# ceselder/pacman-marl-2025

Measured on AMD Instinct MI355X. Metric: env-steps/s (4-agent smallCapture), higher is better.
Workload: dtype u32; 1 GPU; smallCapture.lay 2v2, 16384 envs/GPU, gymPacMan tick (self_play), length 300, auto-reset, uniform random actions (Philox seed 1234), 4 observations/env-tick; envs_per_gpu=16384, layout=smallCapture, obs_dtype=float32, obs_bytes_per_elem=4, parallelism=env-sharded x1, no data-path collective

## Files before the change

### pacman-marl-2025_amd/csrc/pmx_step.hip

```cpp
#include <algorithm>
#include <cstdlib>

#include <hip/hip_ext.h>

#include "pmx_device.h"

#define PMX_MAX_H_LDS 32

namespace {

struct Env {
    uint32_t xy[4];
    int dir[4], pac[4], scared[4], carry[4], ret[4];
    uint32_t capw[2];
    int score, steps;
    uint32_t ticks;
    uint32_t self_after[4];
};

struct Acc {
    double red_r, blue_r;
    int red_sc, blue_sc, sc_total;
    int n_red, n_blue;
};
// ... 475 lines not shown
    st[(size_t)PMX_W_CAPS(c.H, 1) * N + env] = e.capw[1];
}
template <int K0, int K1>
__device__ __forceinline__ void wide_group(const uint32_t *lds_rows, int n_rows, int word0, int sub, int q4, uint32_t *dst, int N)
{
    if constexpr (K0 < K1) {
        const int r = 4 * K0 + sub;
        const uint4 v = *reinterpret_cast<const uint4 *>(lds_rows + (r < n_rows ? r : 0) * PMX_RULE_BLOCK + q4);
        wide_group<K0 + 1, K1>(lds_rows, n_rows, word0, sub, q4, dst, N);
        if (r < n_rows) *reinterpret_cast<uint4 *>(dst + (size_t)(word0 + r) * N) = v;
    }
}
template <int HB, int NW>
__device__ __forceinline__ void store_words_wide(const Ctx &c, const uint32_t (&w)[NW], uint32_t *st, int N)
{
    const int lane = threadIdx.x, sub = lane >> 4, q4 = 4 * (lane & 15);
    uint32_t *dst = st + (size_t)blockIdx.x * PMX_RULE_BLOCK + q4;
#pragma unroll
    for (int i = 0; i < NW; ++i) c.stg[i * PMX_RULE_BLOCK + lane] = w[i];
    __builtin_amdgcn_fence(__ATOMIC_ACQ_REL, "wavefront");
    __builtin_amdgcn_wave_barrier();
    constexpr int KR = HB / 4, KW = (NW + 3) / 4;
    wide_group<0, KR>(c.rows0, c.H, 0, sub, q4, dst, N);
    wide_group<0, KW>(c.stg, NW, c.H, sub, q4, dst, N);
    __builtin_amdgcn_fence(__ATOMIC_ACQ_REL, "wavefront");
    __builtin_amdgcn_wave_barrier();
}
template <int HB>
__device__ __forceinline__ void store_snapshot_wide(const Env &e, const Ctx &c, uint32_t *st, int N)
{
    uint32_t w[10];
#pragma unroll
    for (int i = 0; i < 4; ++i) { w[i] = pack_a(e, i); w[4 + i] = pack_b(e, i); }
    w[8] = e.capw[0]; w[9] = e.capw[1];
    store_words_wide<HB, 10>(c, w, st, N);
}
template <int HB>
__device__ __forceinline__ void store_env_wide(const Env &e, const Ctx &c, uint32_t *st, int N)
{
    uint32_t w[13];
#pragma unroll
    for (int i = 0; i < 4; ++i) { w[i] = pack_a(e, i); w[4 + i] = pack_b(e, i); }
    w[8] = e.capw[0]; w[9] = e.capw[1];
    w[10] = (uint32_t)e.score; w[11] = (uint32_t)e.steps; w[12] = e.ticks;
    store_words_wide<HB, 13>(c, w, st, N);
}
template <int HB = 0>
__device__ __forceinline__ void store_env(const Env &e, const Ctx &c, uint32_t *st, int N, int env)
{
    store_snapshot<HB>(e, c, st, N, env);
    st[(size_t)PMX_W_SCORE(c.H) * N + env] = (uint32_t)e.score;
    st[(size_t)PMX_W_STEPS(c.H) * N + env] = (uint32_t)e.steps;
    st[(size_t)PMX_W_TICKS(c.H) * N + env] = e.ticks;
}
__device__ __forceinline__ int redraw_layout(uint32_t key, uint32_t ticks, int n_layouts)
{
    uint32_t x = key ^ (ticks * 0x85EBCA77u) ^ 0x4C41594Fu;
    x ^= x >> 16; x *= 0x7FEB352Du; x ^= x >> 15; x *= 0x846CA68Bu; x ^= x >> 16;
    return (int)(((uint64_t)x * (uint32_t)n_layouts) >> 32);
}

__device__ __forceinline__ void switch_layout(Ctx &c, const PmxTickParams &p, int env, int li)
{
    p.layout_idx_rw[env] = li;
    c.L = p.lay + li;
#pragma unroll
    for (int i = 0; i < 4; ++i) c.start_xy[i] = (uint32_t)c.L->startx[i] | ((uint32_t)c.L->starty[i] << 8);
    uint32_t *w = const_cast<uint32_t *>(c.wl);
    for (int y = 0; y < 32; ++y) w[y * c.wls] = y < c.H ? c.L->walls[y] : 0xFFFFFFFFu;
}

__device__ __forceinline__ void init_env(Env &e, const Ctx &c)
{
    for (int y = 0; y < c.H; ++y) c.fd[y * PMX_RULE_BLOCK] = c.L->food0[y];
#pragma unroll
    for (int i = 0; i < 4; ++i) {
        e.xy[i] = c.start_xy[i]; e.dir[i] = 4;
        e.pac[i] = 0; e.scared[i] = 0; e.carry[i] = 0; e.ret[i] = 0;
    }
    e.capw[0] = c.L->capw0[0]; e.capw[1] = c.L->capw0[1];
    e.score = 0; e.steps = 0;
}

template <int HB = 0>
__device__ __forceinline__ bool tick_finish(Env &e, Acc &a, const Ctx &c_in, const PmxTickParams &p, int env, bool fused)
{
    Ctx c = c_in;
    double blue_r = a.blue_r + (double)(a.blue_sc > 0 ? a.blue_sc : 0);
    double red_r = a.red_r + (double)(a.red_sc > 0 ? a.red_sc : 0);
    int n_red = 0, n_blue = 0;
    if constexpr (HB > 0) {
        n_red = a.n_red; n_blue = a.n_blue;
    } else {
        for (int y = 0; y < c.H; ++y) {
            uint32_t row = c.fd[y * PMX_RULE_BLOCK];
            n_red += __popc(row & c.lo_mask);
            n_blue += __popc(row & c.hi_mask);
        }
    }
    bool done = (n_blue == 0 && e.carry[0] == 0 && e.carry[2] == 0) ||
                (n_red == 0 && e.carry[1] == 0 && e.carry[3] == 0) || (e.steps >= p.length);
    if (done) {
        const int fs = e.score;
        if (fs < 0) blue_r += 20.0 + (1.0 / 5) * (double)(-fs);
        else if (fs > 0) red_r += 20.0 + (1.0 / 5) * (double)fs;
    }
    e.steps += 1;
    e.ticks += 1;
    if (p.agent_out && fused) {
        uint4 v = make_uint4(e.self_after[0], e.self_after[1], e.self_after[2], e.self_after[3]);
        reinterpret_cast<uint4 *>(p.agent_out)[env] = v;
    }
    if (p.reward) { p.reward[2 * (size_t)env] = red_r; p.reward[2 * (size_t)env + 1] = blue_r; }
    if (p.done) p.done[env] = (uint8_t)done;
    if (p.score_change) p.score_change[env] = a.sc_total;
    if (p.score) p.score[env] = e.score;
    if (done && p.auto_reset) {
        if (p.layout_idx_rw) switch_layout(c, p, env, redraw_layout(c.rng_key, e.ticks, p.n_layouts));
        init_env(e, c);
        const size_t snap_sz = (size_t)PMX_SNAP_WORDS(c.H) * p.N;
        for (int s = 0; s < 3; ++s) store_snapshot(e, c, p.snap + s * snap_sz, p.N, env);
    }
    if (p.legal) {
        uint32_t m = 0;
#pragma unroll
        for (int i = 0; i < 4; ++i) m |= (uint32_t)legal_mask(c.wl, c.wls, (int)(e.xy[i] & 0xFF), (int)(e.xy[i] >> 8)) << (8 * i);
        reinterpret_cast<uint32_t *>(p.legal)[env] = m;
    }
    return done && p.auto_reset;
}

__device__ __forceinline__ Ctx make_ctx_fill(const PmxTickParams &p, uint32_t *lds, const int env0, const unsigned tid)
{
    Ctx c;
    const bool multi = p.layout_idx != nullptr;
    c.L = p.lay + ((multi && env0 < p.N) ? p.layout_idx[env0] : 0);
    c.W = p.lay_W; c.H = p.lay_H; c.half = p.lay_half; c.n_dump = p.lay_n_dump;
    c.dump = p.dump;
    c.legal_reward = p.legal_reward; c.defence_reward = p.defence_reward;
    c.wl = multi ? lds + 32 + PMX_MAX_H_LDS * PMX_RULE_BLOCK + tid : lds;
    c.wls = multi ? PMX_RULE_BLOCK : 1;
    c.fd = lds + 32 + tid;
    c.rows0 = lds + 32;
    c.stg = lds + 32 + (multi ? (3 * PMX_MAX_H_LDS + 32) : 3 * c.H) * PMX_RULE_BLOCK;
    c.fd2 = multi ? lds + 32 + 2 * PMX_MAX_H_LDS * PMX_RULE_BLOCK + tid : lds + 32 + c.H * PMX_RULE_BLOCK + tid;
    c.fd3 = multi ? lds + 32 + 3 * PMX_MAX_H_LDS * PMX_RULE_BLOCK + tid : lds + 32 + 2 * c.H * PMX_RULE_BLOCK + tid;
    c.dist = p.dist ? p.dist + c.L->dist_off : nullptr;
    c.cidx = p.cell_index ? p.cell_index + (size_t)(c.L - p.lay) * 1024 : nullptr;
    c.n_cells = c.L->n_cells;
    c.lo_mask = p.lo_mask; c.hi_mask = p.hi_mask;
#pragma unroll
    for (int i = 0; i < 4; ++i) c.start_xy[i] = (uint32_t)c.L->startx[i] | ((uint32_t)c.L->starty[i] << 8);
    c.rng_key = p.seed ^ ((uint32_t)env0 * 0x9E3779B1u);
    if (tid < 32) lds[tid] = tid < (unsigned)c.H ? p.lay->walls[tid] : 0xFFFFFFFFu;
    if (multi) {
        uint32_t *w = lds + 32 + PMX_MAX_H_LDS * PMX_RULE_BLOCK + tid;
        uint32_t wr[32];
#pragma unroll
        for (int y = 0; y < 32; ++y) wr[y] = y < c.H ? c.L->walls[y] : 0xFFFFFFFFu;
#pragma unroll
        for (int y = 0; y < 32; ++y) w[y * PMX_RULE_BLOCK] = wr[y];
    }
    return c;
}

__device__ __forceinline__ Ctx make_ctx(const PmxTickParams &p, uint32_t *lds)
{
    Ctx c = make_ctx_fill(p, lds, blockIdx.x * PMX_RULE_BLOCK + threadIdx.x, threadIdx.x);
    __syncthreads();
    return c;
}

}

__device__ __forceinline__ void write_walls(const PmxTickParams &p);

template <bool BOTS, int HB>
__global__ __launch_bounds__(PMX_RULE_BLOCK) void pmx_rule_kernel(PmxTickParams p)
{
    extern __shared__ uint32_t lds[];
    if ((int)blockIdx.x >= p.rule_blocks) {
        write_walls(p);
        return;
    }
    const int env = blockIdx.x * PMX_RULE_BLOCK + threadIdx.x;
    const bool live = env < p.N;
    RawEnv raw;
    uint32_t rows[HB];
    uint32_t av = 0;
    if (live) {
        load_env_issue<HB>(raw, rows, p.state, p.N, env, p.lay_H);
        av = reinterpret_cast<const uint32_t *>(p.actions)[env];
    }
    Ctx c = make_ctx(p, lds);
    if (!live) return;
    Env e;
    load_env_commit<HB>(e, c, raw, rows);
    Acc a = { 0.0, 0.0, 0, 0, 0, 0, 0 };
    count_food<HB>(a, c, rows);
    const size_t snap_sz = (size_t)PMX_SNAP_WORDS(c.H) * p.N;
    const bool wide = (p.N & (PMX_RULE_BLOCK - 1)) == 0;
    tick_substep<0, BOTS>(e, a, c, (int)(int8_t)(av & 0xFF));
    if (wide) store_snapshot_wide<HB>(e, c, p.snap, p.N); else store_snapshot<HB>(e, c, p.snap, p.N, env);
    tick_substep<1, BOTS>(e, a, c, (int)(int8_t)((av >> 8) & 0xFF));
// ... 263 lines not shown
    const uint32_t a_self = S[(size_t)PMX_W_AGENT_A(H, agent) * N];
    const uint32_t b_self = S[(size_t)PMX_W_AGENT_B(H, agent) * N];

    const int n_words = (8 * HW + 31) >> 5;
    const int wall_words = (HW + 31) >> 5;
    for (int k = lane; k < n_words + 1; k += 64) T[k] = k < wall_words ? L->wall_stream[k] : 0u;
    __builtin_amdgcn_fence(__ATOMIC_RELEASE, "wavefront");
    __builtin_amdgcn_wave_barrier();
    if (lane < H) {
        stream_or_row(T, (uint32_t)((6 * H + lane) * W), food & L->hi_mask, W);
        stream_or_row(T, (uint32_t)((7 * H + lane) * W), food & L->lo_mask, W);
    }
    if (lane < 4) {
        const int x = pt & 0xFF, y = (pt >> 8) & 0xFF;
        const int plane = lane == agent ? 1 : (((lane ^ agent) == 2) ? 4 : 5);
        const uint32_t off = (uint32_t)((plane * H + y) * W + x);
        atomicOr(&T[off >> 5], 1u << (off & 31));
    } else if (lane < 8) {
        const uint32_t cxy = (pt >> (16 * ((lane - 4) & 1))) & 0xFFFFu;
        if (cxy != 0xFFFFu) {
            const int x = cxy & 0xFF, y = cxy >> 8;
            const int plane = (2 * x > W) ? 2 : 3;
            const uint32_t off = (uint32_t)((plane * H + y) * W + x);
            atomicOr(&T[off >> 5], 1u << (off & 31));
        }
    }
    const uint32_t carry = (b_self >> 8) & 0xFFF;
    const int fself = (H + (int)((a_self >> 8) & 0xFF)) * W + (int)(a_self & 0xFF);
    __builtin_amdgcn_fence(__ATOMIC_ACQ_REL, "wavefront");
    __builtin_amdgcn_wave_barrier();

    const int n_vec = 8 * HW / VEC;
    uint4 *out = reinterpret_cast<uint4 *>(p.obs) + (size_t)q * n_vec;
    for (int k = (BEHIND ? p.first_vec : 0) + lane; k < n_vec; k += 64) {
        const uint32_t e0 = (uint32_t)k * VEC;
        const uint32_t bits = T[e0 >> 5] >> (e0 & 31);
        uint4 v;
        if (DT == 0) v = *reinterpret_cast<const uint4 *>(&lut[(bits & 15u) * 4]);
        else if (DT == 1) v = *reinterpret_cast<const uint4 *>(&lut[(bits & 255u) * 4]);
        else {
            const uint2 lo = *reinterpret_cast<const uint2 *>(&lut[(bits & 255u) * 2]);
            const uint2 hi = *reinterpret_cast<const uint2 *>(&lut[((bits >> 8) & 255u) * 2]);
            v = make_uint4(lo.x, lo.y, hi.x, hi.y);
        }
        const uint32_t d = (uint32_t)(fself - (int)e0);
        if (d < (uint32_t)VEC) patch_self<DT>(v, (int)d, carry);
        if (NT) {
            __builtin_nontemporal_store(v.x, &out[k].x); __builtin_nontemporal_store(v.y, &out[k].y);
            __builtin_nontemporal_store(v.z, &out[k].z); __builtin_nontemporal_store(v.w, &out[k].w);
        } else {
            out[k] = v;
        }
    }
}

#define PMX_FUSED_WAVES 16
__host__ __device__ inline int fused_rule_words(int H) { return 32 + (3 * H + 16) * PMX_RULE_BLOCK; }
__host__ __device__ inline int fused_snap_rows(int H) { return 3 * PMX_SNAP_WORDS(H) + H + 13; }
__host__ __device__ inline int fused_tab_stride(int H, int W) { return (((8 * H * W + 31) >> 5) + 1 + 3) & ~3; }

template <int HB, bool FULL>
__device__ __forceinline__ void snapshot_to_lds(const Env &e, const Ctx &c, uint32_t *slot)
{
    uint32_t rows[HB];
#pragma unroll
    for (int y = 0; y < HB; ++y) rows[y] = y < c.H ? c.fd[y * PMX_RULE_BLOCK] : 0u;
#pragma unroll
    for (int y = 0; y < HB; ++y)
        if (y < c.H) slot[y * PMX_RULE_BLOCK] = rows[y];
#pragma unroll
    for (int i = 0; i < 4; ++i) {
        slot[PMX_W_AGENT_A(c.H, i) * PMX_RULE_BLOCK] = pack_a(e, i);
        slot[PMX_W_AGENT_B(c.H, i) * PMX_RULE_BLOCK] = pack_b(e, i);
    }
    slot[PMX_W_CAPS(c.H, 0) * PMX_RULE_BLOCK] = e.capw[0];
    slot[PMX_W_CAPS(c.H, 1) * PMX_RULE_BLOCK] = e.capw[1];
    if (FULL) {
        slot[PMX_W_SCORE(c.H) * PMX_RULE_BLOCK] = (uint32_t)e.score;
        slot[PMX_W_STEPS(c.H) * PMX_RULE_BLOCK] = (uint32_t)e.steps;
        slot[PMX_W_TICKS(c.H) * PMX_RULE_BLOCK] = e.ticks;
    }
}

template <int HB>
__global__ __launch_bounds__(PMX_FUSED_WAVES * 64) void pmx_tick_fused_kernel(PmxTickParams p, int reverse)
{
    constexpr int VEC = ObsVec<0>::VEC, NB = 4 * PMX_RULE_BLOCK;
    extern __shared__ uint32_t lds[];
    const int wave = __builtin_amdgcn_readfirstlane(threadIdx.x >> 6);
    const int lane = threadIdx.x & 63;
    const int H = p.lay_H, W = p.lay_W, HW = H * W;
    const int group = reverse ? (int)gridDim.x - 1 - (int)blockIdx.x : (int)blockIdx.x;
    uint32_t *snapL = lds + fused_rule_words(H);
    uint32_t *lut = snapL + fused_snap_rows(H) * PMX_RULE_BLOCK;
    uint32_t *wstream = lut + 64;
    uint32_t *T = wstream + 32 + wave * fused_tab_stride(H, W);
    const int slot_words = PMX_SNAP_WORDS(H) * PMX_RULE_BLOCK;
    const int first_vec = HW / VEC, n_vec = 8 * HW / VEC;
    uint4 *obs = reinterpret_cast<uint4 *>(p.obs) + (size_t)group * NB * n_vec;

    if (wave == 0) {
        const int env = group * PMX_RULE_BLOCK + lane;
        RawEnv raw;
        uint32_t rows[HB];
        load_env_issue<HB>(raw, rows, p.state, p.N, env, H);
        const uint32_t av = reinterpret_cast<const uint32_t *>(p.actions)[env];
        Ctx c = make_ctx_fill(p, lds, env, lane);
        __builtin_amdgcn_fence(__ATOMIC_ACQ_REL, "wavefront");
        __builtin_amdgcn_wave_barrier();
        Env e;
        load_env_commit<HB>(e, c, raw, rows);
        Acc a = { 0.0, 0.0, 0, 0, 0, 0, 0 };
        count_food<HB>(a, c, rows);
        uint32_t *col = snapL + lane;
        tick_substep<0, false>(e, a, c, (int)(int8_t)(av & 0xFF));
        snapshot_to_lds<HB, false>(e, c, col);
        tick_substep<1, false>(e, a, c, (int)(int8_t)((av >> 8) & 0xFF));
        snapshot_to_lds<HB, false>(e, c, col + slot_words);
        tick_substep<2, false>(e, a, c, (int)(int8_t)((av >> 16) & 0xFF));
        snapshot_to_lds<HB, false>(e, c, col + 2 * slot_words);
        tick_substep<3, false>(e, a, c, (int)(int8_t)((av >> 24) & 0xFF));
        const bool fresh = tick_finish<HB>(e, a, c, p, env, true);
        snapshot_to_lds<HB, true>(e, c, col + 3 * slot_words);
        if (fresh) {
            for (int s = 0; s < 3; ++s) snapshot_to_lds<HB, false>(e, c, col + s * slot_words);
        }
    } else {
        constexpr int MAXJ = 32 * 32 / VEC / 64;
        if (wave == 1 && lane < 16) *reinterpret_cast<uint4 *>(&lut[4 * lane]) = pack_obs<0>(lane);
        if (wave == 1 && lane < 32) wstream[lane] = p.lay->wall_stream[lane];
        uint4 v[MAXJ];
#pragma unroll
        for (int j = 0; j < MAXJ; ++j) {
            const uint32_t e0 = (uint32_t)(lane + 64 * j) * VEC;
            v[j] = pack_obs<0>(p.lay->wall_stream[e0 >> 5] >> (e0 & 31));
        }
        for (int b = wave - 1; b < NB; b += PMX_FUSED_WAVES - 1) {
            uint4 *out = obs + (size_t)(reverse ? NB - 1 - b : b) * n_vec;
#pragma unroll
            for (int j = 0; j < MAXJ; ++j)
                if (lane + 64 * j < first_vec) {
                    uint4 *o = &out[lane + 64 * j];
                    __builtin_nontemporal_store(v[j].x, &o->x); __builtin_nontemporal_store(v[j].y, &o->y);
                    __builtin_nontemporal_store(v[j].z, &o->z); __builtin_nontemporal_store(v[j].w, &o->w);
                }
        }
    }
    __syncthreads();

    {
        const int n_rows = fused_snap_rows(H), snap_rows = 3 * PMX_SNAP_WORDS(H);
        for (int i = threadIdx.x; i < n_rows * 16; i += PMX_FUSED_WAVES * 64) {
            const int row = i >> 4, q4 = 4 * (i & 15);
            const uint4 w = *reinterpret_cast<const uint4 *>(snapL + row * PMX_RULE_BLOCK + q4);
            uint32_t *dst = row < snap_rows ? p.snap + (size_t)row * p.N : p.state + (size_t)(row - snap_rows) * p.N;
            *reinterpret_cast<uint4 *>(dst + (size_t)group * PMX_RULE_BLOCK + q4) = w;
        }
    }

    const int n_words = (8 * HW + 31) >> 5;
    const uint32_t wallw = lane < 32 ? wstream[lane] : 0u;
    for (int it = 0; it < NB / PMX_FUSED_WAVES; ++it) {
        const int b = it * PMX_FUSED_WAVES + wave;
        const int ql = reverse ? NB - 1 - b : b;
        const int agent = ql & 3;
        const uint32_t *S = snapL + agent * slot_words + (ql >> 2);
        const uint32_t food = lane < H ? S[lane * PMX_RULE_BLOCK] : 0u;
        uint32_t pt = 0;
        if (lane < 4) pt = S[PMX_W_AGENT_A(H, lane) * PMX_RULE_BLOCK];
        else if (lane < 8) pt = S[PMX_W_CAPS(H, (lane - 4) >> 1) * PMX_RULE_BLOCK];
        const uint32_t a_self = S[PMX_W_AGENT_A(H, agent) * PMX_RULE_BLOCK];
        const uint32_t b_self = S[PMX_W_AGENT_B(H, agent) * PMX_RULE_BLOCK];
        for (int k = lane; k < n_words + 1; k += 64) T[k] = k < 32 ? wallw : 0u;
        __builtin_amdgcn_fence(__ATOMIC_RELEASE, "wavefront");
        __builtin_amdgcn_wave_barrier();
        if (lane < H) {
            stream_or_row(T, (uint32_t)((6 * H + lane) * W), food & p.hi_mask, W);
            stream_or_row(T, (uint32_t)((7 * H + lane) * W), food & p.lo_mask, W);
        }
        if (lane < 4) {
            const int x = pt & 0xFF, y = (pt >> 8) & 0xFF;
            const int plane = lane == agent ? 1 : (((lane ^ agent) == 2) ? 4 : 5);
            const uint32_t off = (uint32_t)((plane * H + y) * W + x);
            atomicOr(&T[off >> 5], 1u << (off & 31));
        } else if (lane < 8) {
            const uint32_t cxy = (pt >> (16 * ((lane - 4) & 1))) & 0xFFFFu;
            if (cxy != 0xFFFFu) {
                const int x = cxy & 0xFF, y = cxy >> 8;
                const int plane = (2 * x > W) ? 2 : 3;
                const uint32_t off = (uint32_t)((plane * H + y) * W + x);
                atomicOr(&T[off >> 5], 1u << (off & 31));
            }
        }
        const uint32_t carry = (b_self >> 8) & 0xFFF;
        const int fself = (H + (int)((a_self >> 8) & 0xFF)) * W + (int)(a_self & 0xFF);
        __builtin_amdgcn_fence(__ATOMIC_ACQ_REL, "wavefront");
        __builtin_amdgcn_wave_barrier();

        uint4 *out = obs + (size_t)ql * n_vec;
        for (int k = first_vec + lane; k < n_vec; k += 64) {
            const uint32_t e0 = (uint32_t)k * VEC;
            const uint32_t bits = T[e0 >> 5] >> (e0 & 31);
            uint4 v = *reinterpret_cast<const uint4 *>(&lut[(bits & 15u) * 4]);
            const uint32_t d = (uint32_t)(fself - (int)e0);
            if (d < (uint32_t)VEC) patch_self<0>(v, (int)d, carry);
            out[k] = v;
        }
        __builtin_amdgcn_fence(__ATOMIC_ACQ_REL, "wavefront");
        __builtin_amdgcn_wave_barrier();
    }
}

struct SnapWords { uint32_t food[4], pt[4], a_self[4], b_self[4]; };
__device__ __forceinline__ void load_snap_words(SnapWords &s, const PmxExpandParams &p, long env, int lane, int H)
{
    const size_t N = (size_t)p.N;
#pragma unroll
    for (int a = 0; a < 4; ++a) {
        const uint32_t *S = p.snap[a] + env;
        s.food[a] = lane < H ? S[(size_t)lane * N] : 0u;
        s.pt[a] = 0;
        if (lane < 4) s.pt[a] = S[(size_t)PMX_W_AGENT_A(H, lane) * N];
        else if (lane < 8) s.pt[a] = S[(size_t)PMX_W_CAPS(H, (lane - 4) >> 1) * N];
        s.a_self[a] = S[(size_t)PMX_W_AGENT_A(H, a) * N];
        s.b_self[a] = S[(size_t)PMX_W_AGENT_B(H, a) * N];
    }
}

template <bool NT>
__global__ __launch_bounds__(PMX_BLOCK) void pmx_expand4_kernel(PmxExpandParams p)
{
    constexpr int DT = 2, VEC = ObsVec<DT>::VEC;
    constexpr int TW = 8 * 32 * 32 / 32 + 8;
    __shared__ uint32_t tab[4][4][TW];
    __shared__ __align__(16) uint32_t lut[256 * 2];
    {
        const uint32_t i = threadIdx.x;
        lut[2 * i] = ((i & 15u) * 0x00204081u) & 0x01010101u;
        lut[2 * i + 1] = ((i >> 4) * 0x00204081u) & 0x01010101u;
        __syncthreads();
    }
    const int wave = __builtin_amdgcn_readfirstlane(threadIdx.x >> 6);
    const int lane = threadIdx.x & 63;
    const int W = p.lay_W, H = p.lay_H, HW = H * W;
    long blk = p.reverse ? (long)gridDim.x - 1 - (long)blockIdx.x : (long)blockIdx.x;
    if ((p.N & 127) == 0) {
        const long r = blk & 31;
        blk = (blk & ~31L) + (r & 7) * 4 + (r >> 3);
    }
    const long env = blk * 4 + wave;
    if (env >= p.N) return;
    const int n_words = (8 * HW + 31) >> 5;
    const int wall_words = (HW + 31) >> 5;
    const int n_vec = 8 * HW / VEC;
    SnapWords cur;
    load_snap_words(cur, p, env, lane, H);
    const PmxLayoutDev *L = p.lay + (p.layout_idx ? p.layout_idx[env] : 0);
#pragma unroll
    for (int a = 0; a < 4; ++a)
        for (int k = lane; k < n_words + 1; k += 64) tab[wave][a][k] = k < wall_words ? L->wall_stream[k] : 0u;
    const uint32_t hi_mask = L->hi_mask, lo_mask = L->lo_mask;
    __builtin_amdgcn_fence(__ATOMIC_RELEASE, "wavefront");
    __builtin_amdgcn_wave_barrier();
    int fself[4];
    uint32_t carry[4];
#pragma unroll
    for (int a = 0; a < 4; ++a) {
        uint32_t *T = tab[wave][a];
        if (lane < H) {
            stream_or_row(T, (uint32_t)((6 * H + lane) * W), cur.food[a] & hi_mask, W);
            stream_or_row(T, (uint32_t)((7 * H + lane) * W), cur.food[a] & lo_mask, W);
        }
        if (lane < 4) {
            const int x = cur.pt[a] & 0xFF, y = (cur.pt[a] >> 8) & 0xFF;
            const int plane = lane == a ? 1 : (((lane ^ a) == 2) ? 4 : 5);
            const uint32_t off = (uint32_t)((plane * H + y) * W + x);
            atomicOr(&T[off >> 5], 1u << (off & 31));
        } else if (lane < 8) {
            const uint32_t cxy = (cur.pt[a] >> (16 * ((lane - 4) & 1))) & 0xFFFFu;
            if (cxy != 0xFFFFu) {
                const int x = cxy & 0xFF, y = cxy >> 8;
                const int plane = (2 * x > W) ? 2 : 3;
                const uint32_t off = (uint32_t)((plane * H + y) * W + x);
                atomicOr(&T[off >> 5], 1u << (off & 31));
            }
        }
        carry[a] = (cur.b_self[a] >> 8) & 0xFFF;
        fself[a] = (H + (int)((cur.a_self[a] >> 8) & 0xFF)) * W + (int)(cur.a_self[a] & 0xFF);
    }
    __builtin_amdgcn_fence(__ATOMIC_ACQ_REL, "wavefront");
    __builtin_amdgcn_wave_barrier();

// ... 146 lines not shown
            e0s[u] = ok ? (uint32_t)(kk - s * n_vec) * VEC : 0u;
            bits[u] = (sl[u] == 1 ? T1 : T0)[e0s[u] >> 5] >> (e0s[u] & 31);
            if (sl[u] == 2) {
                const uint32_t d4 = (uint32_t)(f_ally - (int)e0s[u]);
                if (d4 < (uint32_t)VEC) bits[u] &= ~(1u << d4);
                const uint32_t d2 = (uint32_t)(fmate - (int)e0s[u]);
                if (fmate >= 0 && d2 < (uint32_t)VEC) bits[u] |= 1u << d2;
            }
        }
        uint4 v[U];
#pragma unroll
        for (int u = 0; u < U; ++u) {
            if (DT == 0) v[u] = *reinterpret_cast<const uint4 *>(&lut[(bits[u] & 15u) * 4]);
            else if (DT == 1) v[u] = *reinterpret_cast<const uint4 *>(&lut[(bits[u] & 255u) * 4]);
            else {
                const uint2 lo = *reinterpret_cast<const uint2 *>(&lut[(bits[u] & 255u) * 2]);
                const uint2 hi = *reinterpret_cast<const uint2 *>(&lut[((bits[u] >> 8) & 255u) * 2]);
                v[u] = make_uint4(lo.x, lo.y, hi.x, hi.y);
            }
        }
#pragma unroll
        for (int u = 0; u < U; ++u) {
            const int kk = base + 64 * u + lane;
            const int fs = sl[u] == 1 ? fself1 : fself0;
            const uint32_t cr = sl[u] == 0 ? carry0 : (sl[u] == 1 ? carry1 : carry_m);
            const uint32_t d = (uint32_t)(fs - (int)e0s[u]);
            if (d < (uint32_t)VEC) patch_self<DT>(v[u], (int)d, cr);
            if (sl[u] == 2 && fmate >= 0) {
                const uint32_t d2 = (uint32_t)(fmate - (int)e0s[u]);
                if (d2 < (uint32_t)VEC) patch_self<DT>(v[u], (int)d2, carry1);
            }
            if (kk < total) (sl[u] == 2 ? out_merged : out_team)[kk] = v[u];
        }
    }
}

extern "C" hipError_t pmx_launch_emit_team(const PmxEmitParams *p, int dtype, hipStream_t st, hipEvent_t ev0, hipEvent_t ev1)
{
    const unsigned blocks = (unsigned)(((long)p->N + 3) / 4);
#define PMX_EMIT(DT)                                                                                                          \
    do {                                                                                                                      \
        if (ev0) hipExtLaunchKernelGGL(pmx_emit_team_kernel<DT>, dim3(blocks), dim3(PMX_BLOCK), 0, st, ev0, ev1, 0, *p);       \
        else hipLaunchKernelGGL(pmx_emit_team_kernel<DT>, dim3(blocks), dim3(PMX_BLOCK), 0, st, *p);                           \
    } while (0)
    switch (dtype) {
    case 0: PMX_EMIT(0); break;
    case 1: PMX_EMIT(1); break;
    default: PMX_EMIT(2); break;
    }
#undef PMX_EMIT
    return hipGetLastError();
}

extern "C" hipError_t pmx_launch_rule(const PmxTickParams *p, int H, hipStream_t st, hipEvent_t ev0, hipEvent_t ev1)
{
    const int rule_blocks = (p->N + PMX_RULE_BLOCK - 1) / PMX_RULE_BLOCK;
    const size_t lds = (p->layout_idx ? 32 + (size_t)(3 * PMX_MAX_H_LDS + 32 + 16) * PMX_RULE_BLOCK : 32 + (size_t)(3 * H + 16) * PMX_RULE_BLOCK) * sizeof(uint32_t);
    const int hb = H <= 12 ? 12 : (H <= 16 ? 16 : (H <= 20 ? 20 : 32));
    const long obs_blocks = (long)p->N * p->n_emit;
    const int wall_blocks = p->obs ? (int)std::min<long>(obs_blocks, PMX_WALL_BLOCKS) : 0;
    const int blocks = rule_blocks + wall_blocks;
    PmxTickParams q = *p;
    q.rule_blocks = rule_blocks;
#define PMX_RULE_LAUNCH(B, HBV)                                                                                         \
    do {                                                                                                                \
        if (ev0) hipExtLaunchKernelGGL((pmx_rule_kernel<B, HBV>), dim3(blocks), dim3(PMX_RULE_BLOCK), (uint32_t)lds, st, ev0, ev1, 0, q); \
        else hipLaunchKernelGGL((pmx_rule_kernel<B, HBV>), dim3(blocks), dim3(PMX_RULE_BLOCK), lds, st, q);               \
    } while (0)
#define PMX_RULE_PICK(B)                                                                      \
    switch (hb) {                                                                             \
    case 12: PMX_RULE_LAUNCH(B, 12); break;                                                   \
    case 16: PMX_RULE_LAUNCH(B, 16); break;                                                   \
    case 20: PMX_RULE_LAUNCH(B, 20); break;                                                   \
    default: PMX_RULE_LAUNCH(B, 32); break;                                                   \
    }
    if (p->dist) { PMX_RULE_PICK(true) } else { PMX_RULE_PICK(false) }
    return hipGetLastError();
}

extern "C" hipError_t pmx_launch_tick_fused(const PmxTickParams *p, int reverse, hipStream_t st)
{
    const int H = p->lay_H, W = p->lay_W;
    if (H > 20 || (p->N % PMX_RULE_BLOCK) != 0 || p->layout_idx || p->dist || !p->obs || p->n_emit != 4) return hipErrorInvalidValue;
    const size_t lds = ((size_t)fused_rule_words(H) + (size_t)fused_snap_rows(H) * PMX_RULE_BLOCK + 64 + 32 +
                        (size_t)PMX_FUSED_WAVES * fused_tab_stride(H, W)) * sizeof(uint32_t);
    if (lds > ((size_t)64 << 10)) return hipErrorInvalidValue;
    const dim3 grid(p->N / PMX_RULE_BLOCK), block(PMX_FUSED_WAVES * 64);
    if (H <= 12) hipLaunchKernelGGL(pmx_tick_fused_kernel<12>, grid, block, lds, st, *p, reverse);
    else if (H <= 16) hipLaunchKernelGGL(pmx_tick_fused_kernel<16>, grid, block, lds, st, *p, reverse);
    else hipLaunchKernelGGL(pmx_tick_fused_kernel<20>, grid, block, lds, st, *p, reverse);
    return hipGetLastError();
}

extern "C" hipError_t pmx_launch_rule_agent(const PmxTickParams *p, int H, int agent, hipStream_t st)
{
    const int blocks = (p->N + PMX_RULE_BLOCK - 1) / PMX_RULE_BLOCK;
    const size_t lds = (p->layout_idx ? 32 + (size_t)(3 * PMX_MAX_H_LDS + 32 + 16) * PMX_RULE_BLOCK : 32 + (size_t)(3 * H + 16) * PMX_RULE_BLOCK) * sizeof(uint32_t);
    if (p->dist) hipLaunchKernelGGL(pmx_rule_agent_kernel<true>, dim3(blocks), dim3(PMX_RULE_BLOCK), lds, st, *p, agent);
    else hipLaunchKernelGGL(pmx_rule_agent_kernel<false>, dim3(blocks), dim3(PMX_RULE_BLOCK), lds, st, *p, agent);
    return hipGetLastError();
}

extern "C" hipError_t pmx_launch_successor(const PmxTickParams *p, int H, int agent, hipStream_t st)
{
    const int blocks = (p->N + PMX_RULE_BLOCK - 1) / PMX_RULE_BLOCK;
    const size_t lds = (p->layout_idx ? 32 + (size_t)(3 * PMX_MAX_H_LDS + 32 + 16) * PMX_RULE_BLOCK : 32 + (size_t)(3 * H + 16) * PMX_RULE_BLOCK) * sizeof(uint32_t);
    hipLaunchKernelGGL(pmx_successor_kernel, dim3(blocks), dim3(PMX_RULE_BLOCK), lds, st, *p, agent);
    return hipGetLastError();
}

extern "C" hipError_t pmx_launch_bot_query(const PmxTickParams *p, int H, int agent, int code, double *values, int8_t *action,
                                           uint8_t *flags, hipStream_t st)
{
    const int blocks = (p->N + PMX_RULE_BLOCK - 1) / PMX_RULE_BLOCK;
    const size_t lds = (p->layout_idx ? 32 + (size_t)(3 * PMX_MAX_H_LDS + 32 + 16) * PMX_RULE_BLOCK : 32 + (size_t)(3 * H + 16) * PMX_RULE_BLOCK) * sizeof(uint32_t);
    hipLaunchKernelGGL(pmx_bot_query_kernel, dim3(blocks), dim3(PMX_RULE_BLOCK), lds, st, *p, agent, code, values, action, flags);
    return hipGetLastError();
}

extern "C" hipError_t pmx_launch_reset(const PmxTickParams *p, int H, hipStream_t st)
{
    const int blocks = (p->N + PMX_RULE_BLOCK - 1) / PMX_RULE_BLOCK;
    const size_t lds = (p->layout_idx ? 32 + (size_t)(3 * PMX_MAX_H_LDS + 32 + 16) * PMX_RULE_BLOCK : 32 + (size_t)(3 * H + 16) * PMX_RULE_BLOCK) * sizeof(uint32_t);
    hipLaunchKernelGGL(pmx_reset_kernel, dim3(blocks), dim3(PMX_RULE_BLOCK), lds, st, *p);
    return hipGetLastError();
}

extern "C" hipError_t pmx_launch_expand(const PmxExpandParams *p, int dtype, hipStream_t st, hipEvent_t ev0, hipEvent_t ev1)
{
    const long waves = (long)p->N * p->n_emit;
    const unsigned blocks = (unsigned)((waves + 3) / 4);
    const size_t elem = dtype == 0 ? 4 : (dtype == 1 ? 2 : 1);
    const size_t bytes = (size_t)waves * 8 * p->lay_H * p->lay_W * elem;
    const bool nt = elem == 1 || (elem == 2 && bytes > ((size_t)512 << 20)) || (elem == 4 && bytes > PMX_F32_STREAM_BYTES);
    const size_t lds_pad = (nt && elem == 4) ? 40000 : 0;
    PmxExpandParams q = *p;
    if (nt) q.reverse = 0;
    if (dtype == 2 && p->n_emit == 4 && p->single_agent < 0) {
        const unsigned b4 = (unsigned)((p->N + 3) / 4);
        const bool nt4 = bytes > ((size_t)200 << 20);
#define PMX_EXPAND4(NTV)                                                                                                  \
    do {                                                                                                                  \
        if (ev0) hipExtLaunchKernelGGL((pmx_expand4_kernel<NTV>), dim3(b4), dim3(PMX_BLOCK), 0, st, ev0, ev1, 0, q);      \
        else hipLaunchKernelGGL((pmx_expand4_kernel<NTV>), dim3(b4), dim3(PMX_BLOCK), 0, st, q);                          \
    } while (0)
        if (nt4) PMX_EXPAND4(true); else PMX_EXPAND4(false);
#undef PMX_EXPAND4
        return hipGetLastError();
    }
#define PMX_EXPAND(...)                                                                                                 \
    do {                                                                                                                \
        if (ev0) hipExtLaunchKernelGGL((pmx_expand_kernel<__VA_ARGS__>), dim3(blocks), dim3(PMX_BLOCK), (uint32_t)lds_pad, st, ev0, ev1, 0, q); \
        else hipLaunchKernelGGL((pmx_expand_kernel<__VA_ARGS__>), dim3(blocks), dim3(PMX_BLOCK), lds_pad, st, q);       \
    } while (0)
    if (q.first_vec > 0 && (dtype != 0 || nt)) return hipErrorInvalidValue;
    switch (dtype) {
    case 0: if (nt) PMX_EXPAND(0, true); else if (q.first_vec > 0) PMX_EXPAND(0, false, true); else PMX_EXPAND(0, false); break;
    case 1: if (nt) PMX_EXPAND(1, true); else PMX_EXPAND(1, false); break;
    default: PMX_EXPAND(2, true); break;
    }
#undef PMX_EXPAND
    return hipGetLastError();
}
```

Baseline: 313.0 million env-steps/s.

## Overlap agent-0 observation expansion with remaining substeps in fused tick kernel

The fused tick kernel is split into two phases. While wave 0 runs substeps 1-3 and finishes the tick, the other waves already expand agent 0's observations from the substep-0 snapshot. Envs that reset are recorded in a ballot mask, and their agent-0 observations are re-expanded afterwards from the fresh snapshot. The aim is to hide the serial rule-simulation latency of wave 0 behind observation writes, at the cost of an extra block barrier, redundant expansion for reset envs and more complex snapshot bookkeeping.

```diff
diff --git a/pacman-marl-2025_amd/csrc/pmx_step.hip b/pacman-marl-2025_amd/csrc/pmx_step.hip
--- a/pacman-marl-2025_amd/csrc/pmx_step.hip
+++ b/pacman-marl-2025_amd/csrc/pmx_step.hip
@@ -581,7 +581,7 @@
     e.score = 0; e.steps = 0;
 }
 
-template <int HB = 0>
+template <int HB = 0, bool FRESH_SNAP = true>
 __device__ __forceinline__ bool tick_finish(Env &e, Acc &a, const Ctx &c_in, const PmxTickParams &p, int env, bool fused)
 {
     Ctx c = c_in;
@@ -617,8 +617,10 @@
     if (done && p.auto_reset) {
         if (p.layout_idx_rw) switch_layout(c, p, env, redraw_layout(c.rng_key, e.ticks, p.n_layouts));
         init_env(e, c);
-        const size_t snap_sz = (size_t)PMX_SNAP_WORDS(c.H) * p.N;
-        for (int s = 0; s < 3; ++s) store_snapshot(e, c, p.snap + s * snap_sz, p.N, env);
+        if constexpr (FRESH_SNAP) {
+            const size_t snap_sz = (size_t)PMX_SNAP_WORDS(c.H) * p.N;
+            for (int s = 0; s < 3; ++s) store_snapshot(e, c, p.snap + s * snap_sz, p.N, env);
+        }
     }
     if (p.legal) {
         uint32_t m = 0;
@@ -1048,6 +1050,56 @@
     }
 }
 
+__device__ __forceinline__ void fused_expand_block(const PmxTickParams &p, const uint32_t *S, int agent, uint32_t *T, const uint32_t *lut,
+                                                   uint32_t wallw, uint4 *out, int lane)
+{
+    constexpr int VEC = ObsVec<0>::VEC;
+    const int H = p.lay_H, W = p.lay_W, HW = H * W;
+    const int first_vec = HW / VEC, n_vec = 8 * HW / VEC, n_words = (8 * HW + 31) >> 5;
+    const uint32_t food = lane < H ? S[lane * PMX_RULE_BLOCK] : 0u;
+    uint32_t pt = 0;
+    if (lane < 4) pt = S[PMX_W_AGENT_A(H, lane) * PMX_RULE_BLOCK];
+    else if (lane < 8) pt = S[PMX_W_CAPS(H, (lane - 4) >> 1) * PMX_RULE_BLOCK];
+    const uint32_t a_self = S[PMX_W_AGENT_A(H, agent) * PMX_RULE_BLOCK];
+    const uint32_t b_self = S[PMX_W_AGENT_B(H, agent) * PMX_RULE_BLOCK];
+    for (int k = lane; k < n_words + 1; k += 64) T[k] = k < 32 ? wallw : 0u;
+    __builtin_amdgcn_fence(__ATOMIC_RELEASE, "wavefront");
+    __builtin_amdgcn_wave_barrier();
+    if (lane < H) {
+        stream_or_row(T, (uint32_t)((6 * H + lane) * W), food & p.hi_mask, W);
+        stream_or_row(T, (uint32_t)((7 * H + lane) * W), food & p.lo_mask, W);
+    }
+    if (lane < 4) {
+        const int x = pt & 0xFF, y = (pt >> 8) & 0xFF;
+        const int plane = lane == agent ? 1 : (((lane ^ agent) == 2) ? 4 : 5);
+        const uint32_t off = (uint32_t)((plane * H + y) * W + x);
+        atomicOr(&T[off >> 5], 1u << (off & 31));
+    } else if (lane < 8) {
+        const uint32_t cxy = (pt >> (16 * ((lane - 4) & 1))) & 0xFFFFu;
+        if (cxy != 0xFFFFu) {
+            const int x = cxy & 0xFF, y = cxy >> 8;
+            const int plane = (2 * x > W) ? 2 : 3;
+            const uint32_t off = (uint32_t)((plane * H + y) * W + x);
+            atomicOr(&T[off >> 5], 1u << (off & 31));
+        }
+    }
+    const uint32_t carry = (b_self >> 8) & 0xFFF;
+    const int fself = (H + (int)((a_self >> 8) & 0xFF)) * W + (int)(a_self & 0xFF);
+    __builtin_amdgcn_fence(__ATOMIC_ACQ_REL, "wavefront");
+    __builtin_amdgcn_wave_barrier();
+
+    for (int k = first_vec + lane; k < n_vec; k += 64) {
+        const uint32_t e0 = (uint32_t)k * VEC;
+        const uint32_t bits = T[e0 >> 5] >> (e0 & 31);
+        uint4 v = *reinterpret_cast<const uint4 *>(&lut[(bits & 15u) * 4]);
+        const uint32_t d = (uint32_t)(fself - (int)e0);
+        if (d < (uint32_t)VEC) patch_self<0>(v, (int)d, carry);
+        out[k] = v;
+    }
+    __builtin_amdgcn_fence(__ATOMIC_ACQ_REL, "wavefront");
+    __builtin_amdgcn_wave_barrier();
+}
+
 template <int HB>
 __global__ __launch_bounds__(PMX_FUSED_WAVES * 64) void pmx_tick_fused_kernel(PmxTickParams p, int reverse)
 {
@@ -1060,37 +1112,31 @@
     uint32_t *snapL = lds + fused_rule_words(H);
     uint32_t *lut = snapL + fused_snap_rows(H) * PMX_RULE_BLOCK;
     uint32_t *wstream = lut + 64;
-    uint32_t *T = wstream + 32 + wave * fused_tab_stride(H, W);
+    uint32_t *freshL = wstream + 32;
+    uint32_t *T = freshL + 4 + wave * fused_tab_stride(H, W);
     const int slot_words = PMX_SNAP_WORDS(H) * PMX_RULE_BLOCK;
     const int first_vec = HW / VEC, n_vec = 8 * HW / VEC;
     uint4 *obs = reinterpret_cast<uint4 *>(p.obs) + (size_t)group * NB * n_vec;
+    const int env = group * PMX_RULE_BLOCK + lane;
+
+    Env e;
+    Acc a = { 0.0, 0.0, 0, 0, 0, 0, 0 };
+    Ctx c;
+    uint32_t av = 0;
+    uint32_t *col = snapL + lane;
 
     if (wave == 0) {
-        const int env = group * PMX_RULE_BLOCK + lane;
         RawEnv raw;
         uint32_t rows[HB];
         load_env_issue<HB>(raw, rows, p.state, p.N, env, H);
-        const uint32_t av = reinterpret_cast<const uint32_t *>(p.actions)[env];
-        Ctx c = make_ctx_fill(p, lds, env, lane);
+        av = reinterpret_cast<const uint32_t *>(p.actions)[env];
+        c = make_ctx_fill(p, lds, env, lane);
         __builtin_amdgcn_fence(__ATOMIC_ACQ_REL, "wavefront");
         __builtin_amdgcn_wave_barrier();
-        Env e;
         load_env_commit<HB>(e, c, raw, rows);
-        Acc a = { 0.0, 0.0, 0, 0, 0, 0, 0 };
         count_food<HB>(a, c, rows);
-        uint32_t *col = snapL + lane;
         tick_substep<0, false>(e, a, c, (int)(int8_t)(av & 0xFF));
         snapshot_to_lds<HB, false>(e, c, col);
-        tick_substep<1, false>(e, a, c, (int)(int8_t)((av >> 8) & 0xFF));
-        snapshot_to_lds<HB, false>(e, c, col + slot_words);
-        tick_substep<2, false>(e, a, c, (int)(int8_t)((av >> 16) & 0xFF));
-        snapshot_to_lds<HB, false>(e, c, col + 2 * slot_words);
-        tick_substep<3, false>(e, a, c, (int)(int8_t)((av >> 24) & 0xFF));
-        const bool fresh = tick_finish<HB>(e, a, c, p, env, true);
-        snapshot_to_lds<HB, true>(e, c, col + 3 * slot_words);
-        if (fresh) {
-            for (int s = 0; s < 3; ++s) snapshot_to_lds<HB, false>(e, c, col + s * slot_words);
-        }
     } else {
         constexpr int MAXJ = 32 * 32 / VEC / 64;
         if (wave == 1 && lane < 16) *reinterpret_cast<uint4 *>(&lut[4 * lane]) = pack_obs<0>(lane);
@@ -1114,9 +1160,42 @@
     }
     __syncthreads();
 
+    const uint32_t wallw = lane < 32 ? wstream[lane] : 0u;
+    if (wave == 0) {
+        tick_substep<1, false>(e, a, c, (int)(int8_t)((av >> 8) & 0xFF));
+        snapshot_to_lds<HB, false>(e, c, col + slot_words);
+        tick_substep<2, false>(e, a, c, (int)(int8_t)((av >> 16) & 0xFF));
+        snapshot_to_lds<HB, false>(e, c, col + 2 * slot_words);
+        tick_substep<3, false>(e, a, c, (int)(int8_t)((av >> 24) & 0xFF));
+        const bool fresh = tick_finish<HB, false>(e, a, c, p, env, true);
+        snapshot_to_lds<HB, true>(e, c, col + 3 * slot_words);
+        if (fresh) {
+            snapshot_to_lds<HB, false>(e, c, col + slot_words);
+            snapshot_to_lds<HB, false>(e, c, col + 2 * slot_words);
+        }
+        const unsigned long long fb = __ballot(fresh);
+        if (lane == 0) { freshL[0] = (uint32_t)fb; freshL[1] = (uint32_t)(fb >> 32); }
+    } else {
+        for (int j = wave - 1; j < PMX_RULE_BLOCK; j += PMX_FUSED_WAVES - 1) {
+            const int el = reverse ? PMX_RULE_BLOCK - 1 - j : j;
+            fused_expand_block(p, snapL + el, 0, T, lut, wallw, obs + (size_t)(4 * el) * n_vec, lane);
+        }
+    }
+    __syncthreads();
+
     {
-        const int n_rows = fused_snap_rows(H), snap_rows = 3 * PMX_SNAP_WORDS(H);
-        for (int i = threadIdx.x; i < n_rows * 16; i += PMX_FUSED_WAVES * 64) {
+        const int n_rows = fused_snap_rows(H), rows0 = PMX_SNAP_WORDS(H), snap_rows = 3 * rows0;
+        int i, i_end, i_step;
+        if (wave == 0) {
+            if ((lane < 32 ? freshL[0] >> lane : freshL[1] >> (lane - 32)) & 1u)
+                for (int r = 0; r < rows0; ++r) col[r * PMX_RULE_BLOCK] = col[slot_words + r * PMX_RULE_BLOCK];
+            __builtin_amdgcn_fence(__ATOMIC_ACQ_REL, "wavefront");
+            __builtin_amdgcn_wave_barrier();
+            i = lane; i_end = rows0 * 16; i_step = 64;
+        } else {
+            i = rows0 * 16 + (int)threadIdx.x - 64; i_end = n_rows * 16; i_step = (PMX_FUSED_WAVES - 1) * 64;
+        }
+        for (; i < i_end; i += i_step) {
             const int row = i >> 4, q4 = 4 * (i & 15);
             const uint4 w = *reinterpret_cast<const uint4 *>(snapL + row * PMX_RULE_BLOCK + q4);
             uint32_t *dst = row < snap_rows ? p.snap + (size_t)row * p.N : p.state + (size_t)(row - snap_rows) * p.N;
@@ -1124,56 +1203,21 @@
         }
     }
 
-    const int n_words = (8 * HW + 31) >> 5;
-    const uint32_t wallw = lane < 32 ? wstream[lane] : 0u;
-    for (int it = 0; it < NB / PMX_FUSED_WAVES; ++it) {
+    const uint32_t fresh_lo = __builtin_amdgcn_readfirstlane(freshL[0]), fresh_hi = __builtin_amdgcn_readfirstlane(freshL[1]);
+    if (wave != 0 && (fresh_lo | fresh_hi) != 0u) {
+        for (int j = wave - 1; j < PMX_RULE_BLOCK; j += PMX_FUSED_WAVES - 1) {
+            const int el = reverse ? PMX_RULE_BLOCK - 1 - j : j;
+            if (((el < 32 ? fresh_lo >> el : fresh_hi >> (el - 32)) & 1u) == 0u) continue;
+            fused_expand_block(p, snapL + slot_words + el, 0, T, lut, wallw, obs + (size_t)(4 * el) * n_vec, lane);
+        }
+    }
+
+    constexpr int NB3 = 3 * PMX_RULE_BLOCK;
+    for (int it = 0; it < NB3 / PMX_FUSED_WAVES; ++it) {
         const int b = it * PMX_FUSED_WAVES + wave;
-        const int ql = reverse ? NB - 1 - b : b;
-        const int agent = ql & 3;
-        const uint32_t *S = snapL + agent * slot_words + (ql >> 2);
-        const uint32_t food = lane < H ? S[lane * PMX_RULE_BLOCK] : 0u;
-        uint32_t pt = 0;
-        if (lane < 4) pt = S[PMX_W_AGENT_A(H, lane) * PMX_RULE_BLOCK];
-        else if (lane < 8) pt = S[PMX_W_CAPS(H, (lane - 4) >> 1) * PMX_RULE_BLOCK];
-        const uint32_t a_self = S[PMX_W_AGENT_A(H, agent) * PMX_RULE_BLOCK];
-        const uint32_t b_self = S[PMX_W_AGENT_B(H, agent) * PMX_RULE_BLOCK];
-        for (int k = lane; k < n_words + 1; k += 64) T[k] = k < 32 ? wallw : 0u;
-        __builtin_amdgcn_fence(__ATOMIC_RELEASE, "wavefront");
-        __builtin_amdgcn_wave_barrier();
-        if (lane < H) {
-            stream_or_row(T, (uint32_t)((6 * H + lane) * W), food & p.hi_mask, W);
-            stream_or_row(T, (uint32_t)((7 * H + lane) * W), food & p.lo_mask, W);
-        }
-        if (lane < 4) {
-            const int x = pt & 0xFF, y = (pt >> 8) & 0xFF;
-            const int plane = lane == agent ? 1 : (((lane ^ agent) == 2) ? 4 : 5);
-            const uint32_t off = (uint32_t)((plane * H + y) * W + x);
-            atomicOr(&T[off >> 5], 1u << (off & 31));
-        } else if (lane < 8) {
-            const uint32_t cxy = (pt >> (16 * ((lane - 4) & 1))) & 0xFFFFu;
-            if (cxy != 0xFFFFu) {
-                const int x = cxy & 0xFF, y = cxy >> 8;
-                const int plane = (2 * x > W) ? 2 : 3;
-                const uint32_t off = (uint32_t)((plane * H + y) * W + x);
-                atomicOr(&T[off >> 5], 1u << (off & 31));
-            }
-        }
-        const uint32_t carry = (b_self >> 8) & 0xFFF;
-        const int fself = (H + (int)((a_self >> 8) & 0xFF)) * W + (int)(a_self & 0xFF);
-        __builtin_amdgcn_fence(__ATOMIC_ACQ_REL, "wavefront");
-        __builtin_amdgcn_wave_barrier();
-
-        uint4 *out = obs + (size_t)ql * n_vec;
-        for (int k = first_vec + lane; k < n_vec; k += 64) {
-            const uint32_t e0 = (uint32_t)k * VEC;
-            const uint32_t bits = T[e0 >> 5] >> (e0 & 31);
-            uint4 v = *reinterpret_cast<const uint4 *>(&lut[(bits & 15u) * 4]);
-            const uint32_t d = (uint32_t)(fself - (int)e0);
-            if (d < (uint32_t)VEC) patch_self<0>(v, (int)d, carry);
-            out[k] = v;
-        }
-        __builtin_amdgcn_fence(__ATOMIC_ACQ_REL, "wavefront");
-        __builtin_amdgcn_wave_barrier();
+        const int m = reverse ? NB3 - 1 - b : b;
+        const int el = m / 3, agent = 1 + m - 3 * el;
+        fused_expand_block(p, snapL + agent * slot_words + el, agent, T, lut, wallw, obs + (size_t)(4 * el + agent) * n_vec, lane);
     }
 }
 
@@ -1486,7 +1530,7 @@
 {
     const int H = p->lay_H, W = p->lay_W;
     if (H > 20 || (p->N % PMX_RULE_BLOCK) != 0 || p->layout_idx || p->dist || !p->obs || p->n_emit != 4) return hipErrorInvalidValue;
-    const size_t lds = ((size_t)fused_rule_words(H) + (size_t)fused_snap_rows(H) * PMX_RULE_BLOCK + 64 + 32 +
+    const size_t lds = ((size_t)fused_rule_words(H) + (size_t)fused_snap_rows(H) * PMX_RULE_BLOCK + 64 + 32 + 4 +
                         (size_t)PMX_FUSED_WAVES * fused_tab_stride(H, W)) * sizeof(uint32_t);
     if (lds > ((size_t)64 << 10)) return hipErrorInvalidValue;
     const dim3 grid(p->N / PMX_RULE_BLOCK), block(PMX_FUSED_WAVES * 64);
```

Result: faster. 323.2 million env-steps/s (median of 6 runs) (+3.3%).
